# outbrain-inc/fwumious_wabbit

Measured on AMD Instinct MI355X. Metric: examples/sec + final log-loss, 30-field k=8 FFM, at 1/2/4/8 MI355X, higher is better.
Workload: dtype f32

## Files before the change

fwumious_wabbit_amd/_capi.py:

```python
import ctypes as C
import os

import numpy as np

_HERE = os.path.dirname(os.path.abspath(__file__))
LIB_PATH = os.environ.get("FWGPU_LIBRARY") or os.path.join(_HERE, "lib", "libfwgpu.so")

OK = 0
ERR_INVALID = 1
ERR_RANGE = 4
ERR_PARSE, ERR_IO, PARSE_FLUSH, PARSE_HOGWILD_LOAD = 6, 7, 100, 101
FFM_F32, FFM_F16_BUCKETS = 0, 1
OPT_SGD, OPT_ADAGRAD_FLEX, OPT_ADAGRAD_LUT = 100, 200, 300
WIRING_REGRESSOR, WIRING_FFM_ONLY = 0, 1
MODE_SEQUENTIAL, MODE_HOGWILD = 0, 1
TABLE_LR, TABLE_FFM_W, TABLE_FFM_ACC, TABLE_NN_W, TABLE_NN_ACC = 0, 1, 2, 3, 4
ROUTE_NONE, ROUTE_FUSED, ROUTE_HEAD_BATCHED, ROUTE_HEAD_BATCHED_REFUSED, ROUTE_PACKED, ROUTE_HOST_WALK = 0, 1, 2, 3, 4, 5
NN_INIT = {"xavier": 0, "hu": 1, "one": 2, "zero": 3}

CANDIDATE_INFO = np.dtype([("code", "<i4"), ("is_delta", "u1"), ("record_ok", "u1"), ("by_host", "u1"), ("pad", "u1"), ("n_lr", "<u4"),
                           ("n_ffm", "<u4")])
LR_ENTRY = np.dtype([("hash", "<u4"), ("value", "<f4"), ("combo_index", "<u4")])
FFM_ENTRY = np.dtype([("hash", "<u4"), ("value", "<f4"), ("contra_field_index", "<u4")])

# ... 106 lines not shown
        "fwgpu_dist_group_set_mode": [vp, i32],
        "fwgpu_dist_rank": [vp, P(i32), P(i32)],
        "fwgpu_dist_comm_count": [vp, P(i32)],
        "fwgpu_dist_ranges": [vp, P(u32), P(u32), P(u32), P(u32)],
        "fwgpu_dist_learn_sharded": [vp, P(TranslatorConfig), vp, vp, u32, vp],
        "fwgpu_dist_learn_sharded_batch": [vp, P(TranslatorConfig), vp],
        "fwgpu_dist_gather_tables": [vp],
        "fwgpu_dist_all_reduce_sum": [vp, vp, u64, vp],
        "fwgpu_dist_group_create": [vp, i32, P(vp)],
        "fwgpu_dist_group_free": [vp],
        "fwgpu_dist_group_learn_sharded": [vp, P(TranslatorConfig), vp, vp, u32, vp],
        "fwgpu_dist_group_gather_tables": [vp],
        "fwgpu_dist_learn_sparse": [vp, P(TranslatorConfig), vp, vp, u32, vp],
        "fwgpu_dist_learn_sparse_batch": [vp, P(TranslatorConfig), vp],
        "fwgpu_dist_sparse_last_rows": [vp, P(u32), P(u32)],
        "fwgpu_dist_group_learn_sparse": [vp, P(TranslatorConfig), vp, vp, vp, vp],
        "fwgpu_dist_group_learn_peer": [vp, P(TranslatorConfig), vp, vp, vp, vp, i32],
        "fwgpu_dist_peer_attach": [vp],
        "fwgpu_dist_owner_attach": [vp, u32, u32],
        "fwgpu_dist_learn_owner": [vp, P(TranslatorConfig), vp, vp, u32, vp, i32],
        "fwgpu_dist_group_learn_owner": [vp, P(TranslatorConfig), vp, vp, vp, vp, i32],
        "fwgpu_dist_group_learn_owner_stream": [vp, P(TranslatorConfig), vp, vp, vp, vp, vp, i32, u32, u32, u32],
        "fwgpu_dist_owner_stream_attach": [vp, u32, u32],
        "fwgpu_dist_learn_owner_stream": [vp, P(TranslatorConfig), vp, vp, u32, vp, i32, u32],
        "fwgpu_dist_learn_peer": [vp, P(TranslatorConfig), vp, vp, u32, vp, i32],
        "fwgpu_dist_learn_peer_batch": [vp, P(TranslatorConfig), vp, i32, vp],
        "fwgpu_dist_barrier": [vp],
        "fwgpu_split_create": [vp, u32, u32, P(vp)],
        "fwgpu_split_free": [vp],
        "fwgpu_learn_batch_sync": [vp, vp, vp, i32, vp],
        "fwgpu_serialized_len": [vp, P(u64)],
        "fwgpu_write_weights": [vp, vp, u64, P(u64)],
        "fwgpu_read_weights": [vp, vp, u64],
        "fwgpu_table_len": [vp, i32, P(u64)],
        "fwgpu_table_read": [vp, i32, u64, u64, vp],
        "fwgpu_table_write": [vp, i32, u64, u64, vp],
        "fwgpu_table_fill": [vp, i32, f32],
        "fwgpu_table_checksum": [vp, i32, P(u64)],
        "fwgpu_table_device_ptr": [vp, i32, P(vp)],
        "fwgpu_batch_create": [vp, vp, vp, vp, vp, vp, vp, u32, P(vp)],
        "fwgpu_batch_free": [vp],
        "fwgpu_batch_size": [vp, P(u32), P(u64), P(u64)],
        "fwgpu_learn_batch": [vp, vp, i32, i32, vp],
        "fwgpu_batch_predictions": [vp, vp, u32, vp],
        "fwgpu_batch_predictions_device": [vp, P(vp)],
        "fwgpu_translate": [P(TranslatorConfig), vp, u32, vp, u32, P(u32), vp, u32, P(u32), P(f32), P(f32)],
        "fwgpu_batch_from_records": [vp, P(TranslatorConfig), vp, vp, u32, P(vp)],
        "fwgpu_record_batch_create": [vp, P(TranslatorConfig), vp, vp, u32, P(vp)],
        "fwgpu_trainer_create": [vp, P(TranslatorConfig), u32, P(vp)],
        "fwgpu_digest_records": [vp, vp, vp, u32],
        "fwgpu_finish": [vp],
        "fwgpu_trainer_free": [vp],
        "fwgpu_trainer_examples_seen": [vp, P(u64)],
        "fwgpu_trainer_set_holdout": [vp, u64, i32],
        "fwgpu_trainer_predictions": [vp, vp, u64, P(u64)],
        "fwgpu_set_launch": [vp, u32, u32],
        "fwgpu_set_max_in_flight": [vp, u32],
        "fwgpu_delta_start": [vp, vp, vp, vp, u64, f32, vp],
        "fwgpu_delta_finish": [vp, vp, vp, vp, u64, vp],
        "fwgpu_debug_phase_ticks": [vp, i32, vp],
        "fwgpu_debug_placement": [vp, P(i32), P(C.c_float), P(C.c_float)],
        "fwgpu_debug_set_kernel_version": [vp, i32],
        "fwgpu_debug_set_option": [vp, i32, i32],
        "fwgpu_debug_last_route": [vp, P(i32)],
        "fwgpu_debug_head_inputs": [vp, vp, u64],
        "fwgpu_debug_coherence_probe": [i32, i32, u32, P(u32), P(u32)],
        "fwgpu_debug_head_gemm": [vp, vp, vp, i32, i32, i32, i32, i32, i32, i32, i32, i32, vp, vp, i32, i32, vp],
        "fwgpu_debug_sparse_reduce": [vp, u32, i32, vp, u32, u32, u32, vp, u32, vp, u32, vp, vp, vp, P(u32), vp],
        "fwgpu_debug_sparse_apply": [vp, vp, vp, u32, u32, i32, u32, u32, vp, vp, i32, f32, f32, vp, vp],
        "fwgpu_synth_records": [P(SynthConfig), u64, u32, vp, u64, vp, P(u64)],
        "fwgpu_debug_format_f32": [f32, C.c_char_p, u32],
        "fwgpu_vwmap_from_csv": [C.c_char_p, u64, P(vp)],
        "fwgpu_vwmap_from_json": [C.c_char_p, u64, P(vp)],
        "fwgpu_vwmap_to_json": [vp, vp, u64, P(u64)],
        "fwgpu_vwmap_lookup": [vp, C.c_char_p, u64, i32, P(u32), P(u32)],
        "fwgpu_parser_create": [vp, P(vp)],
        "fwgpu_parser_parse_line": [vp, C.c_char_p, u64, vp, u32, P(u32)],
        "fwgpu_parser_parse_with_prefix": [vp, C.c_char_p, u64, C.c_char_p, u64, vp, u32, P(u32)],
        "fwgpu_parse_prefix_create": [vp, C.c_char_p, u64, P(vp)],
        "fwgpu_parse_prefix_resumable": [vp],
        "fwgpu_parser_parse_after_prefix": [vp, vp, C.c_char_p, u64, vp, u32, P(u32)],
        "fwgpu_parse_prefix_is_record": [vp, vp, u32],
        "fwgpu_parser_parse_candidate": [vp, vp, C.c_char_p, u64, vp, u32, P(u32), P(i32)],
        "fwgpu_parser_parse_buffer": [vp, C.c_char_p, u64, vp, u64, vp, u64, P(u64), P(u64), P(u64)],
        "fwgpu_text_parser_create": [vp, i32, P(vp)],
        "fwgpu_text_parser_parse_buffer": [vp, C.c_char_p, u64, vp, u64, vp, u64, P(u64), P(u64), P(u64)],
        "fwgpu_text_parser_last_lines": [vp, P(u64), P(u64)],
        "fwgpu_text_parser_parse_candidates": [vp, vp, vp, P(TranslatorConfig), C.c_char_p, u64, u64, vp, u64, vp, vp, P(u64), P(u64)],
        "fwgpu_record_batch_from_text": [vp, P(TranslatorConfig), vp, C.c_char_p, u64, u64, P(vp), P(u64), P(u64)],
        "fwgpu_f32_from_text": [C.c_char_p, u64, P(f32), P(i32)],
        "fwgpu_mi_from_json": [C.c_char_p, u64, P(vp)],
        "fwgpu_mi_to_json": [vp, vp, u64, P(u64)],
        "fwgpu_mi_configs": [vp, i32, P(Config), P(TranslatorConfig), P(NNConfig)],
        "fwgpu_mi_set_inference": [vp, i32],
        "fwgpu_model_save": [C.c_char_p, vp, vp, vp, i32],
        "fwgpu_model_read_header": [C.c_char_p, P(vp), P(vp)],
        "fwgpu_model_load": [C.c_char_p, i32, i32, P(vp), P(vp), P(vp)],
        "fwgpu_model_load_packed": [C.c_char_p, i32, P(vp), P(vp), P(vp)],
        "fwgpu_ffm_storage": [vp, P(i32), P(u64)],
        "fwgpu_set_wiring": [vp, i32],
        "fwgpu_model_convert_inference": [C.c_char_p, C.c_char_p, i32],
        "fwgpu_quantize_ffm_weights": [vp, u64, vp, u64],
        "fwgpu_dequantize_ffm_weights": [vp, u64, vp],
        "fwgpu_trainer_digest_cache": [vp, vp, u64, P(u64)],
        "fwgpu_trainer_digest_text": [vp, vp, vp, C.c_char_p, u64, u32, P(u64), P(u64)],
        "fwgpu_parser_clone": [vp, P(vp)],
# ... 47 lines not shown
```

fwumious_wabbit_amd/csrc/fwgpu_internal.h:

```cpp
#pragma once

#include <hip/hip_runtime.h>
#include <stdint.h>

#include <memory>
#include <string>
#include <condition_variable>
#include <functional>
#include <mutex>
#include <thread>
#include <vector>

#include "fwgpu.h"

namespace fwgpu {

constexpr int kLutBits = 11;
constexpr int kLutSize = 1 << kLutBits;
constexpr uint32_t kFfmContraBufLen = 41472;

void set_error(const std::string &msg);
int fail(int code, const std::string &msg);
#define FWGPU_HIP(call)                                                                                  \
    do {                                                                                                 \
// ... 461 lines not shown
                 uint32_t *n_lr, uint32_t *n_ffm);
struct TextLines {
    const fwgpu_candidate_info *info = nullptr;
    const uint64_t *rec_off = nullptr;
    uint64_t n_lines = 0, n_words = 0;
};
int text_lines_scan(fwgpu_text_parser *tp, const fwgpu_parse_prefix *px, const fwgpu_block_cache *cache, const fwgpu_translator_config *t,
                    const char *text, uint64_t len, uint64_t piece_bytes, bool zero_word1, TextLines *out);
int text_lines_place(fwgpu_text_parser *tp, uint32_t *d_records);
int record_batch_alloc(fwgpu_regressor *r, const fwgpu_translator_config *t, uint32_t n_cap, uint64_t words_cap,
                       fwgpu_batch **out, bool host_mapped = false);
int mapped_batch_next_counter(fwgpu_batch *b, hipStream_t stream);
constexpr uint32_t kWorkRing = 1024;
struct RecordStats {
    uint32_t max_lr = 0, max_ffm = 0, max_rec = 0;
    uint64_t tot_lr = 0, tot_ffm = 0;
    void merge(const RecordStats &o) {
        max_lr = max_lr > o.max_lr ? max_lr : o.max_lr;
        max_ffm = max_ffm > o.max_ffm ? max_ffm : o.max_ffm;
        max_rec = max_rec > o.max_rec ? max_rec : o.max_rec;
        tot_lr += o.tot_lr;
        tot_ffm += o.tot_ffm;
    }
};
int count_records(const fwgpu_translator_config *t, const uint32_t *records, const uint64_t *rec_off, uint32_t n,
                  RecordStats *st);
int record_batch_upload(fwgpu_batch *b, const fwgpu_translator_config *t, const uint32_t *records,
                        const uint64_t *rec_off, uint32_t n, hipStream_t stream, const RecordStats *stats = nullptr);
uint32_t lr_hash_mask(uint32_t bit_precision);
uint32_t ffm_hash_mask(uint32_t ffm_bits, uint32_t ffm_k);
void lut_init(float *lut, float learning_rate, float power_t, float init_acc);
KernelParams make_params(const fwgpu_regressor *r, const fwgpu_batch *b, int update);
int refuse_packed(const fwgpu_regressor *r, const char *what);
int create_packed(const fwgpu_config *cfg, const float *lr_w, const uint8_t *blob, fwgpu_regressor **out);
int run_batch_peer(fwgpu_regressor *r, fwgpu_batch *b, int mode, int update, const PeerShards *d_shards, hipStream_t stream,
                   const PushRings *d_push = nullptr, uint32_t stream_consumers = 0, uint32_t device_share = 1, uint32_t stream_max_consumer_waves = 0, uint32_t n_ranks = 0);
hipError_t launch_rendezvous(uint32_t *counter, uint32_t n, uint32_t *met, hipStream_t stream);
hipError_t launch_owner_apply(const fwgpu_regressor *r, float *lr_base, const uint32_t *keys, const float *rows, uint32_t n_rows, const uint2 *lr_ent,
                              uint32_t n_lr, bool in_order, hipStream_t stream);
struct SplitRanges {
    uint32_t ffm_lo = 0, ffm_hi = 0xffffffffu, lr_lo = 0, lr_hi = 0xffffffffu, home_lo = 0, home_hi = 0xffffffffu;
};
struct OccBuffers {
    unsigned long long *ffm_key = nullptr, *lr_key = nullptr;
    uint2 *ffm_desc = nullptr, *lr_desc = nullptr;
};
int split_forward(fwgpu_regressor *r, fwgpu_batch *b, fwgpu_split *sp, int mode, const SplitRanges &rg, hipStream_t stream,
                  const OccBuffers *occ = nullptr, uint32_t *max_ffm = nullptr, uint32_t *max_lr = nullptr);
int split_mid(fwgpu_regressor *r, fwgpu_split *sp, uint32_t first, uint32_t n, float *d_pred, bool head, hipStream_t stream);
int split_update(fwgpu_regressor *r, fwgpu_batch *b, fwgpu_split *sp, int mode, const SplitRanges &rg, bool head, hipStream_t stream);
int head_step(fwgpu_regressor *r, fwgpu_split *sp, uint32_t first, uint32_t n, float *d_pred, bool update, hipStream_t stream);
void head_scratch_free(fwgpu_regressor *r);
uint32_t pick_grid(const fwgpu_regressor *r, const KernelParams &p, int mode, uint32_t threads);
}
```

fwumious_wabbit_amd/csrc/regressor.cpp:

```cpp
#include <math.h>
#include <string.h>

#include <algorithm>
#include <memory>

#include "fwgpu_internal.h"

#ifndef FWGPU_LR_THIN_DEFAULT
#define FWGPU_LR_THIN_DEFAULT 1
#endif
namespace fwgpu {

static thread_local std::string g_last_error;
void set_error(const std::string &msg) { g_last_error = msg; }
int fail(int code, const std::string &msg) {
    g_last_error = msg;
    return code;
}

int refuse_packed(const fwgpu_regressor *r, const char *what) {
    if (!r || !r->packed()) return FWGPU_OK;
    return fail(FWGPU_ERR_INVALID, std::string(what) + ": the regressor's FFM weights are packed f16 buckets (fwgpu_model_load_packed): it only predicts");
}

// ... 463 lines not shown
    if (!b->aligned4)
        return fail(FWGPU_ERR_INVALID, "packed regressor: an FFM entry's hash is not a multiple of 4 (rows must start where the translator's mask puts them: hash & fwgpu_ffm_hash_mask)");
    KernelParams p;
    uint32_t threads = 0;
    const int32_t kv = r->launch.kernel_version;
    r->launch.kernel_version = 0;
    int rc = prepare_launch(r, b, mode, 0, p, threads);
    r->launch.kernel_version = kv;
    if (rc) return rc;
    if (!example_kernel_is_resident(p, threads))
        return fail(FWGPU_ERR_INVALID, "packed regressor: the launch shape is not served (workgroups of at most 512 threads, at most 2048 FFM features per example)");
    const uint32_t grid = pick_grid(r, p, mode, threads);
    if (b->work_ring) {
        rc = mapped_batch_next_counter(b, stream);
        if (rc) return rc;
        p.work = b->work;
    } else {
        FWGPU_HIP(hipMemsetAsync(b->work, 0, sizeof(uint32_t), stream));
    }
    FWGPU_HIP(launch_packed_predict(p, r->q_increment, r->q_min, grid, threads, stream));
    return FWGPU_OK;
}

static int run_batch(fwgpu_regressor *r, fwgpu_batch *b, int mode, int update, hipStream_t stream, int32_t *route = nullptr) {
    if (route) *route = FWGPU_ROUTE_PACKED;
    if (r->packed()) return run_batch_packed(r, b, mode, update, stream);
    if (route) *route = FWGPU_ROUTE_NONE;
    if (b->n == 0) return FWGPU_OK;
    if (route) *route = FWGPU_ROUTE_HOST_WALK;
    if (b->host_copy) return run_batch_by_example(r, b, update, stream);
    if (route) *route = FWGPU_ROUTE_FUSED;
    if (head_predict_batched(r, b, mode, update)) {
        const int rcb = run_batch_head_predict(r, b, stream);
        if (route) *route = rcb == FWGPU_ERR_RANGE ? FWGPU_ROUTE_HEAD_BATCHED_REFUSED : FWGPU_ROUTE_HEAD_BATCHED;
        if (rcb != FWGPU_ERR_RANGE) {
            if (route && rcb == FWGPU_OK) r->pred_n = b->n;
            return rcb;
        }
    }
    KernelParams p;
    uint32_t threads = 0;
    int rc = prepare_launch(r, b, mode, update, p, threads);
    if (rc) return rc;
    const uint32_t grid = pick_grid(r, p, mode, threads);
    if (b->work_ring) {
        rc = mapped_batch_next_counter(b, stream);
        if (rc) return rc;
        p.work = b->work;
    } else {
        FWGPU_HIP(hipMemsetAsync(b->work, 0, sizeof(uint32_t), stream));
    }
    FWGPU_HIP(launch_example_kernel(p, r->cfg.optimizer, update != 0, grid, threads, stream));
    return FWGPU_OK;
}

static constexpr uint32_t kHeadPredictSlab = 32768;
static bool head_predict_batched(const fwgpu_regressor *r, const fwgpu_batch *b, int mode, int update) {
    static const bool env_off = getenv("FWGPU_HEAD_PREDICT_PER_EXAMPLE") != nullptr;
    const bool off = r->launch.head_predict >= 0 ? r->launch.head_predict == 0 : env_off;
    if (off || update || !r->nn.n_layers || mode != FWGPU_MODE_HOGWILD || b->n < 256 || b->emit_T) return false;
    const uint32_t k = r->cfg.ffm_k, R = k * r->cfg.ffm_num_fields;
    return k && k % 4 == 0 && b->aligned4 && (R <= 256 || (R <= 512 && 256 % k == 0)) && r->launch.kernel_version != 1;
}
static int run_batch_head_predict(fwgpu_regressor *r, fwgpu_batch *b, hipStream_t stream) {
    const uint32_t X = r->nn.X;
    if (r->pred_cap < b->n) {
        FWGPU_HIP(hipStreamSynchronize(stream));
        if (r->pred_x) (void)hipFree(r->pred_x);
        if (r->pred_yi) (void)hipFree(r->pred_yi);
        r->pred_x = r->pred_yi = nullptr;
        r->pred_cap = 0;
        if (hipMalloc((void **)&r->pred_x, (size_t)b->n * X * sizeof(float)) != hipSuccess || hipMalloc((void **)&r->pred_yi, (size_t)b->n * 2 * sizeof(float)) != hipSuccess) {
            (void)hipGetLastError();
            return fail(FWGPU_ERR_OOM, "predict batch with a deep head: no memory for the head's inputs");
        }
        r->pred_cap = b->n;
    }
    KernelParams p;
    uint32_t threads = 0;
    {
        p = make_params(r, b, 0);
        if (p.ctx_rec && b->max_rec < p.ctx_rec_len) return fail(FWGPU_ERR_RANGE, "candidate-only records: the batch's longest record does not include the context's");
        p.emit_x = 1;
        p.xbuf = r->pred_x;
        p.gbuf = r->pred_yi;
        threads = std::min<uint32_t>(r->launch.threads, 512);
        if ((uint64_t)p.max_ffm > 4ull * threads) return fail(FWGPU_ERR_RANGE, "an example has more than 2048 FFM features");
        resolve_row_mode(p, threads);
        if (example_kernel_lds_bytes(p, r->cfg.optimizer) > r->lds_per_cu) return fail(FWGPU_ERR_RANGE, "example does not fit the LDS");
    }
    if (b->work_ring) {
        int rc = mapped_batch_next_counter(b, stream);
        if (rc) return rc;
        p.work = b->work;
    } else {
        FWGPU_HIP(hipMemsetAsync(b->work, 0, sizeof(uint32_t), stream));
    }
    FWGPU_HIP(launch_example_kernel(p, r->cfg.optimizer, false, 0, threads, stream));
    fwgpu_split view;
    view.owner = r;
    view.d_x = r->pred_x;
    view.d_g = r->pred_yi;
    for (uint32_t first = 0; first < b->n; first += kHeadPredictSlab) {
        int rc = head_step(r, &view, first, std::min(kHeadPredictSlab, b->n - first), b->pred + first, false, stream);
        if (rc) return rc;
    }
// ... 1315 lines not shown
```

fwumious_wabbit_amd/csrc/trainer.cpp:

```cpp
#include <string.h>

#include <string>

#include <algorithm>
#include <memory>
#include <chrono>
#include <thread>

#include "fwgpu_internal.h"

using namespace fwgpu;

struct fwgpu_trainer {
    fwgpu_regressor *r = nullptr;
    uint32_t micro_batch = 0;
    std::vector<uint32_t> combo_off, combo_ns, field_off, field_ns;
    std::vector<uint8_t> combo_f32, field_f32;
    std::vector<float> combo_weight;
    fwgpu_translator_config t{};
    uint32_t *rec[2] = {nullptr, nullptr};
    uint64_t rec_used[2] = {0, 0}, rec_cap[2] = {0, 0};
    std::vector<uint64_t> off[2];
    RecordStats stats[2];
    unsigned host_threads = 1;
    fwgpu_batch *dev[2] = {nullptr, nullptr};
    hipEvent_t done[2] = {nullptr, nullptr};
    hipEvent_t uploaded[2] = {nullptr, nullptr};
    hipStream_t copy_stream = nullptr;
    bool in_flight[2] = {false, false};
    int cur = 0;
    hipStream_t stream = nullptr;
    uint64_t seen = 0;
    uint64_t holdout_after = 0;
    bool testonly = false;
    bool slot_predict[2] = {false, false};
    uint32_t slot_n[2] = {0, 0};
    float *pred_host[2] = {nullptr, nullptr};
    uint32_t pred_cap[2] = {0, 0};
    std::vector<float> preds;
    std::unique_ptr<uint32_t[]> cache_words[2];
    std::unique_ptr<uint64_t[]> cache_off[2];
    uint64_t cache_off_cap = 0;
    Workers copy_pool, parse_pool;
};

static bool predict_mode(const fwgpu_trainer *tr) {
    return tr->testonly || (tr->holdout_after && tr->seen + 1 >= tr->holdout_after);
}

static int retire(fwgpu_trainer *tr, int c) {
    if (!tr->in_flight[c]) return FWGPU_OK;
    FWGPU_HIP(hipEventSynchronize(tr->done[c]));
    tr->in_flight[c] = false;
    if (tr->slot_predict[c]) tr->preds.insert(tr->preds.end(), tr->pred_host[c], tr->pred_host[c] + tr->slot_n[c]);
    tr->slot_predict[c] = false;
    return FWGPU_OK;
}

static int flush(fwgpu_trainer *tr, bool predict = false) {
    const int c = tr->cur;
    const uint32_t n = (uint32_t)(tr->off[c].size() - 1);
    if (n == 0) return FWGPU_OK;
    fwgpu_regressor *r = tr->r;
    FWGPU_HIP(hipSetDevice(r->device));
    int rrc = retire(tr, c);
    if (rrc) return rrc;
    const uint64_t words = tr->rec_used[c];
    fwgpu_batch *b = tr->dev[c];
    if (!b || b->n_cap < n || b->words_cap < words) {
        if (b) fwgpu_batch_free(b);
        tr->dev[c] = nullptr;
        int rc = record_batch_alloc(r, &tr->t, std::max(n, tr->micro_batch), words * 3 / 2 + 4096, &tr->dev[c]);
        if (rc) return rc;
        b = tr->dev[c];
    }
    int rc = record_batch_upload(b, &tr->t, tr->rec[c], tr->off[c].data(), n, tr->copy_stream, &tr->stats[c]);
    if (rc) return rc;
    if ((rc = record_batch_host_copy_if_oversize(r, &tr->t, b, tr->rec[c], tr->off[c].data(), n))) return rc;
    FWGPU_HIP(hipEventRecord(tr->uploaded[c], tr->copy_stream));
    FWGPU_HIP(hipStreamWaitEvent(tr->stream, tr->uploaded[c], 0));
    rc = fwgpu_learn_batch(r, b, FWGPU_MODE_HOGWILD, predict ? 0 : 1, tr->stream);
    if (rc) return rc;
    if (predict) {
        if (tr->pred_cap[c] < n) {
            if (tr->pred_host[c]) (void)hipHostFree(tr->pred_host[c]);
            tr->pred_host[c] = nullptr;
            FWGPU_HIP(hipHostMalloc((void **)&tr->pred_host[c], (size_t)std::max(n, tr->micro_batch) * 4, hipHostMallocDefault));
            tr->pred_cap[c] = std::max(n, tr->micro_batch);
        }
        FWGPU_HIP(hipMemcpyAsync(tr->pred_host[c], b->pred, (size_t)n * 4, hipMemcpyDeviceToHost, tr->stream));
    }
    tr->slot_predict[c] = predict;
    tr->slot_n[c] = n;
    FWGPU_HIP(hipEventRecord(tr->done[c], tr->stream));
    tr->in_flight[c] = true;
    tr->cur ^= 1;
    const int c2 = tr->cur;
    rrc = retire(tr, c2);
    if (rrc) return rrc;
    tr->rec_used[c2] = 0;
    tr->off[c2].assign(1, 0);
    tr->stats[c2] = RecordStats();
    return FWGPU_OK;
}

extern "C" {

int fwgpu_trainer_create(fwgpu_regressor *r, const fwgpu_translator_config *t, uint32_t micro_batch, fwgpu_trainer **out) {
    if (!r || !t || !out) return fail(FWGPU_ERR_INVALID, "NULL argument");
    if (micro_batch == 0) return fail(FWGPU_ERR_INVALID, "micro_batch must be > 0");
    if (int rcp = refuse_packed(r, "trainer_create")) return rcp;
    int crc = check_translator(r, t);
    if (crc) return crc;
    std::unique_ptr<fwgpu_trainer> tr(new fwgpu_trainer());
    tr->r = r;
    tr->micro_batch = micro_batch;
    tr->combo_off.assign(t->combo_off, t->combo_off + t->n_combos + 1);
    const uint32_t ncm = t->n_combos ? t->combo_off[t->n_combos] : 0;
    tr->combo_ns.assign(t->combo_ns, t->combo_ns + ncm);
    tr->combo_f32.assign(t->combo_ns_f32, t->combo_ns_f32 + ncm);
    tr->combo_weight.assign(t->combo_weight, t->combo_weight + t->n_combos);
    tr->field_off.assign(t->field_off, t->field_off + t->n_fields + 1);
    const uint32_t nfm = t->n_fields ? t->field_off[t->n_fields] : 0;
    tr->field_ns.assign(t->field_ns, t->field_ns + nfm);
    tr->field_f32.assign(t->field_ns_f32, t->field_ns_f32 + nfm);
    tr->t = *t;
    tr->t.combo_off = tr->combo_off.data();
    tr->t.combo_ns = tr->combo_ns.data();
    tr->t.combo_ns_f32 = tr->combo_f32.data();
    tr->t.combo_weight = tr->combo_weight.data();
    tr->t.field_off = tr->field_off.data();
    tr->t.field_ns = tr->field_ns.data();
    tr->t.field_ns_f32 = tr->field_f32.data();
    tr->off[0].assign(1, 0);
    tr->off[1].assign(1, 0);
    tr->host_threads = std::max(1u, std::thread::hardware_concurrency());
    FWGPU_HIP(hipSetDevice(r->device));
    FWGPU_HIP(hipStreamCreateWithFlags(&tr->stream, hipStreamNonBlocking));
    FWGPU_HIP(hipStreamCreateWithFlags(&tr->copy_stream, hipStreamNonBlocking));
    FWGPU_HIP(hipEventCreateWithFlags(&tr->uploaded[0], hipEventDisableTiming));
    FWGPU_HIP(hipEventCreateWithFlags(&tr->uploaded[1], hipEventDisableTiming));
    FWGPU_HIP(hipEventCreateWithFlags(&tr->done[0], hipEventDisableTiming));
    FWGPU_HIP(hipEventCreateWithFlags(&tr->done[1], hipEventDisableTiming));
    *out = tr.release();
    return FWGPU_OK;
}

int fwgpu_digest_records(fwgpu_trainer *tr, const uint32_t *records, const uint64_t *rec_off, uint32_t n) {
    if (!tr || (n && (!records || !rec_off))) return fail(FWGPU_ERR_INVALID, "NULL argument");
    uint32_t i = 0;
    while (i < n) {
        const int c = tr->cur;
        const uint32_t have = (uint32_t)(tr->off[c].size() - 1);
        uint32_t take = std::min<uint32_t>(n - i, tr->micro_batch - have);
        const bool predicting = predict_mode(tr);
        if (!predicting && tr->holdout_after) {
            const uint64_t until = tr->holdout_after - 1 - tr->seen;
            if (take > until) take = (uint32_t)until;
        }
        const uint64_t w0 = rec_off[i], w1 = rec_off[i + take];
        const uint64_t base = tr->rec_used[c];
        if (base + (w1 - w0) > tr->rec_cap[c]) {
            const uint64_t ncap = std::max<uint64_t>((base + (w1 - w0)) * 2, 1u << 20);
            uint32_t *nbuf = nullptr;
            FWGPU_HIP(hipSetDevice(tr->r->device));
            FWGPU_HIP(hipHostMalloc((void **)&nbuf, ncap * 4, hipHostMallocDefault));
            if (base) memcpy(nbuf, tr->rec[c], base * 4);
            if (tr->rec[c]) (void)hipHostFree(tr->rec[c]);
            tr->rec[c] = nbuf;
            tr->rec_cap[c] = ncap;
        }
        {
            const unsigned T = take >= 4096 ? std::min<unsigned>(tr->host_threads, 8) : 1;
            std::vector<RecordStats> st(T);
            std::vector<int> rcs(T, FWGPU_OK);
            std::vector<std::string> msgs(T);
            auto work = [&](unsigned k) {
                const uint32_t a = i + (uint32_t)((uint64_t)take * k / T), e = i + (uint32_t)((uint64_t)take * (k + 1) / T);
                memcpy(tr->rec[c] + base + (rec_off[a] - w0), records + rec_off[a], (rec_off[e] - rec_off[a]) * 4);
                rcs[k] = count_records(&tr->t, records, rec_off + a, e - a, &st[k]);
                if (rcs[k]) msgs[k] = fwgpu_last_error();
            };
            tr->copy_pool.run(T, work);
            for (unsigned k = 0; k < T; k++) {
                if (rcs[k]) return fail(rcs[k], msgs[k]);
                tr->stats[c].merge(st[k]);
            }
        }
        tr->rec_used[c] = base + (w1 - w0);
        for (uint32_t j = 1; j <= take; j++) tr->off[c].push_back(base + (rec_off[i + j] - w0));
        tr->seen += take;
        i += take;
        if (tr->off[c].size() - 1 >= tr->micro_batch || (!predicting && predict_mode(tr))) {
            int rc = flush(tr, predicting);
// ... 193 lines not shown
    auto ms = [](std::chrono::steady_clock::time_point a, std::chrono::steady_clock::time_point b) {
        return std::chrono::duration<double, std::milli>(b - a).count();
    };
    while (have) {
        bool go_on = true;
        double t_digest = 0.0;
        const auto t0 = now();
        std::thread dg([&] {
            go_on = digest_slices(cur, rc, msg);
            t_digest = ms(t0, now());
        });
        bool parsed_next = false;
        if (pos < len) {
            const uint64_t e = chunk_end(pos);
            parse_range(pos, e, next);
            pos = e;
            parsed_next = true;
        }
        const double t_parse = ms(t0, now());
        dg.join();
        if (timing) fprintf(stderr, "[digest_text] chunk: parse of the next %.2f ms, digest of this one %.2f ms, both %.2f ms\n", t_parse, t_digest, ms(t0, now()));
        if (!go_on || !parsed_next) break;
        cur.swap(next);
    }
    if (rc != FWGPU_OK && rc != FWGPU_PARSE_FLUSH && rc != FWGPU_PARSE_HOGWILD_LOAD) rc = fail(rc, msg);
    if (n_examples) *n_examples = done;
    if (consumed) *consumed = used;
    return rc;
}

int fwgpu_trainer_set_holdout(fwgpu_trainer *tr, uint64_t holdout_after, int testonly) {
    if (!tr) return fail(FWGPU_ERR_INVALID, "NULL trainer");
    if (tr->off[tr->cur].size() > 1) return fail(FWGPU_ERR_INVALID, "set the hold-out before digesting (or right after fwgpu_finish)");
    tr->holdout_after = holdout_after;
    tr->testonly = testonly != 0;
    return FWGPU_OK;
}

int fwgpu_trainer_predictions(fwgpu_trainer *tr, float *out, uint64_t cap, uint64_t *n) {
    if (!tr || !n) return fail(FWGPU_ERR_INVALID, "NULL argument");
    *n = tr->preds.size();
    if (!out) return FWGPU_OK;
    if (cap < tr->preds.size()) return fail(FWGPU_ERR_RANGE, "buffer too small for the predictions");
    if (!tr->preds.empty()) memcpy(out, tr->preds.data(), tr->preds.size() * 4);
    return FWGPU_OK;
}

int fwgpu_finish(fwgpu_trainer *tr) {
    if (!tr) return fail(FWGPU_ERR_INVALID, "NULL trainer");
    const bool last_predict = tr->testonly || (tr->holdout_after && tr->seen >= tr->holdout_after);
    int rc = flush(tr, last_predict);
    if (rc) return rc;
    FWGPU_HIP(hipSetDevice(tr->r->device));
    FWGPU_HIP(hipStreamSynchronize(tr->stream));
    rc = retire(tr, tr->cur);
    if (rc) return rc;
    rc = retire(tr, tr->cur ^ 1);
    if (rc) return rc;
    return FWGPU_OK;
}

int fwgpu_trainer_free(fwgpu_trainer *tr) {
    if (!tr) return FWGPU_OK;
    (void)hipSetDevice(tr->r->device);
    if (tr->stream) (void)hipStreamSynchronize(tr->stream);
    for (int i = 0; i < 2; i++) {
        if (tr->dev[i]) fwgpu_batch_free(tr->dev[i]);
        if (tr->rec[i]) (void)hipHostFree(tr->rec[i]);
        if (tr->pred_host[i]) (void)hipHostFree(tr->pred_host[i]);
        if (tr->done[i]) (void)hipEventDestroy(tr->done[i]);
    }
    if (tr->stream) (void)hipStreamDestroy(tr->stream);
    if (tr->copy_stream) (void)hipStreamDestroy(tr->copy_stream);
    for (int i = 0; i < 2; i++)
        if (tr->uploaded[i]) (void)hipEventDestroy(tr->uploaded[i]);
    delete tr;
    return FWGPU_OK;
}

int fwgpu_trainer_examples_seen(const fwgpu_trainer *tr, uint64_t *n) {
    if (!tr || !n) return fail(FWGPU_ERR_INVALID, "NULL argument");
    *n = tr->seen;
    return FWGPU_OK;
}

}
```

fwumious_wabbit_amd/regressor.py:

```python
import ctypes as C
from dataclasses import dataclass, field
from typing import List, Optional, Tuple

import numpy as np

from . import _capi as capi
from ._capi import FFM_ENTRY, LR_ENTRY, check, ptr


class Optimizer:
    SGD = capi.OPT_SGD
    AdagradFlex = capi.OPT_ADAGRAD_FLEX
    AdagradLUT = capi.OPT_ADAGRAD_LUT


@dataclass
class NamespaceDescriptor:
    namespace_index: int
    namespace_format_f32: bool = False


@dataclass
class FeatureComboDesc:
    namespace_descriptors: List[NamespaceDescriptor]
# ... 456 lines not shown
        self.translator = FeatureBufferTranslator(model_instance)
        self.h = C.c_void_p()
        check(capi.lib().fwgpu_trainer_create(regressor.h, C.byref(self.translator.c), micro_batch, C.byref(self.h)))

    def digest_example(self, feature_buffer):
        rec = np.ascontiguousarray(feature_buffer, dtype=np.uint32)
        off = np.array([0, len(rec)], dtype=np.uint64)
        check(capi.lib().fwgpu_digest_records(self.h, ptr(rec), ptr(off), 1))

    def digest_records(self, records, rec_off):
        records = np.ascontiguousarray(records, dtype=np.uint32)
        rec_off = np.ascontiguousarray(rec_off, dtype=np.uint64)
        check(capi.lib().fwgpu_digest_records(self.h, ptr(records), ptr(rec_off), len(rec_off) - 1))

    def set_holdout(self, holdout_after=0, testonly=False):
        check(capi.lib().fwgpu_trainer_set_holdout(self.h, holdout_after, int(testonly)))

    def predictions(self) -> np.ndarray:
        n = C.c_uint64()
        check(capi.lib().fwgpu_trainer_predictions(self.h, None, 0, C.byref(n)))
        out = np.zeros(n.value, dtype=np.float32)
        check(capi.lib().fwgpu_trainer_predictions(self.h, ptr(out), out.size, C.byref(n)))
        return out

    def digest_cache(self, cache, max_records=0) -> int:
        n = C.c_uint64()
        check(capi.lib().fwgpu_trainer_digest_cache(self.h, cache.h, max_records, C.byref(n)))
        return n.value

    def digest_text(self, parser, text: bytes, cache=None, threads=0):
        n, used = C.c_uint64(), C.c_uint64()
        rc = capi.lib().fwgpu_trainer_digest_text(self.h, parser.h, cache.h if cache is not None else None, text, len(text),
                                                  threads, C.byref(n), C.byref(used))
        if rc not in (capi.OK, capi.PARSE_FLUSH, capi.PARSE_HOGWILD_LOAD):
            check(rc)
        return n.value, used.value, rc

    def digest_file(self, parser, filename: str, cache=None, threads=0):
        n = C.c_uint64()
        rc = capi.lib().fwgpu_trainer_digest_file(self.h, parser.h, cache.h if cache is not None else None, filename.encode(),
                                                  threads, C.byref(n))
        if rc not in (capi.OK, capi.PARSE_FLUSH, capi.PARSE_HOGWILD_LOAD):
            check(rc)
        return n.value, rc

    def block_until_workers_finished(self):
        check(capi.lib().fwgpu_finish(self.h))

    def examples_seen(self):
        n = C.c_uint64(0)
        check(capi.lib().fwgpu_trainer_examples_seen(self.h, C.byref(n)))
        return n.value

    def close(self):
        if self.h:
            capi.lib().fwgpu_trainer_free(self.h)
            self.h = C.c_void_p()

    def __del__(self):
        try:
            self.close()
        except Exception:
            pass


def synth_records(n_namespaces, mean_extra, zipf_s, ids_per_ns, p_weighted, seed, first_example, n):
    L = capi.lib()
    cfg = capi.SynthConfig(n_namespaces, mean_extra, zipf_s, ids_per_ns, p_weighted, seed)
    nw = C.c_uint64(0)
    rec_off = np.zeros(n + 1, dtype=np.uint64)
    check(L.fwgpu_synth_records(C.byref(cfg), first_example, n, None, 0, ptr(rec_off), C.byref(nw)))
    records = np.zeros(nw.value, dtype=np.uint32)
    check(L.fwgpu_synth_records(C.byref(cfg), first_example, n, ptr(records), nw.value, ptr(rec_off), C.byref(nw)))
    return records, rec_off
```

include/fwgpu.h:

```cpp
#ifndef FWGPU_H
#define FWGPU_H

#include <stddef.h>
#include <stdint.h>

#ifdef __cplusplus
extern "C" {
#endif

#define FWGPU_ABI_VERSION 1

enum {
    FWGPU_OK = 0,
    FWGPU_ERR_INVALID = 1,
    FWGPU_ERR_DEVICE = 2,
    FWGPU_ERR_OOM = 3,
    FWGPU_ERR_RANGE = 4,
    FWGPU_ERR_FORMAT = 5,
    FWGPU_ERR_PARSE = 6,
    FWGPU_ERR_IO = 7,
    FWGPU_ERR_PEER = 8,
    FWGPU_PARSE_FLUSH = 100,
    FWGPU_PARSE_HOGWILD_LOAD = 101
};
// ... 127 lines not shown

typedef struct fwgpu_dist fwgpu_dist;
typedef struct fwgpu_dist_group fwgpu_dist_group;
int fwgpu_dist_unique_id(uint8_t *id, uint64_t cap );
int fwgpu_dist_init(fwgpu_regressor *r, const uint8_t *unique_id, int rank, int n_ranks, fwgpu_dist **out);
int fwgpu_dist_free(fwgpu_dist *d);
int fwgpu_dist_set_mode(fwgpu_dist *d, int mode);
int fwgpu_dist_group_set_mode(fwgpu_dist_group *g, int mode);
int fwgpu_dist_owner_attach(fwgpu_dist *d, uint32_t max_rows, uint32_t max_lr);
int fwgpu_dist_learn_owner(fwgpu_dist *d, const fwgpu_translator_config *t, const uint32_t *records, const uint64_t *rec_off, uint32_t n,
                           float *predictions, int update);
int fwgpu_dist_group_learn_owner(fwgpu_dist_group *g, const fwgpu_translator_config *t, const uint32_t *const *records,
                                 const uint64_t *const *rec_off, const uint32_t *n, float *const *predictions, int update);
int fwgpu_dist_group_learn_owner_stream(fwgpu_dist_group *g, const fwgpu_translator_config *t, const uint32_t *const *records, const uint64_t *const *rec_off,
                                        const uint32_t *n, fwgpu_batch *const *batches, float *const *predictions, int update, uint32_t log2_rows,
                                        uint32_t log2_lr, uint32_t consumer_workgroups);
int fwgpu_dist_owner_stream_attach(fwgpu_dist *d, uint32_t log2_rows, uint32_t log2_lr);
int fwgpu_dist_learn_owner_stream(fwgpu_dist *d, const fwgpu_translator_config *t, const uint32_t *records, const uint64_t *rec_off, uint32_t n,
                                  float *predictions, int update, uint32_t consumer_workgroups);
int fwgpu_dist_rank(const fwgpu_dist *d, int *rank, int *n_ranks);
int fwgpu_dist_comm_count(const fwgpu_dist *d, int *count);
int fwgpu_dist_ranges(const fwgpu_dist *d, uint32_t *ffm_lo, uint32_t *ffm_hi, uint32_t *lr_lo, uint32_t *lr_hi);
int fwgpu_dist_learn_sharded(fwgpu_dist *d, const fwgpu_translator_config *t, const uint32_t *records, const uint64_t *rec_off,
                             uint32_t n, float *predictions);
int fwgpu_dist_learn_sharded_batch(fwgpu_dist *d, const fwgpu_translator_config *t, fwgpu_batch *b);
int fwgpu_dist_gather_tables(fwgpu_dist *d);
int fwgpu_dist_all_reduce_sum(fwgpu_dist *d, float *device_buf, uint64_t count, void *hip_stream);
int fwgpu_dist_group_create(fwgpu_regressor *const *regressors, int n_ranks, fwgpu_dist_group **out);
int fwgpu_dist_group_free(fwgpu_dist_group *g);
int fwgpu_dist_group_learn_sharded(fwgpu_dist_group *g, const fwgpu_translator_config *t, const uint32_t *const *records,
                                   const uint64_t *const *rec_off, uint32_t n, float *const *predictions);
int fwgpu_dist_group_gather_tables(fwgpu_dist_group *g);
int fwgpu_dist_learn_sparse(fwgpu_dist *d, const fwgpu_translator_config *t, const uint32_t *records, const uint64_t *rec_off,
                            uint32_t n, float *predictions);
int fwgpu_dist_learn_sparse_batch(fwgpu_dist *d, const fwgpu_translator_config *t, fwgpu_batch *b);
int fwgpu_dist_sparse_last_rows(const fwgpu_dist *d, uint32_t *ffm_rows, uint32_t *lr_rows);
int fwgpu_dist_group_learn_sparse(fwgpu_dist_group *g, const fwgpu_translator_config *t, const uint32_t *const *records,
                                  const uint64_t *const *rec_off, const uint32_t *n, float *const *predictions);
int fwgpu_dist_group_learn_peer(fwgpu_dist_group *g, const fwgpu_translator_config *t, const uint32_t *const *records,
                                const uint64_t *const *rec_off, const uint32_t *n, float *const *predictions, int update);
int fwgpu_dist_peer_attach(fwgpu_dist *d);
int fwgpu_dist_learn_peer(fwgpu_dist *d, const fwgpu_translator_config *t, const uint32_t *records, const uint64_t *rec_off, uint32_t n,
                          float *predictions, int update);
int fwgpu_dist_learn_peer_batch(fwgpu_dist *d, const fwgpu_translator_config *t, fwgpu_batch *b, int update, void *hip_stream);
int fwgpu_dist_barrier(fwgpu_dist *d);


int fwgpu_trainer_create(fwgpu_regressor *r, const fwgpu_translator_config *t, uint32_t micro_batch,
                         fwgpu_trainer **out);
int fwgpu_digest_records(fwgpu_trainer *tr, const uint32_t *records, const uint64_t *rec_off, uint32_t n);
int fwgpu_finish(fwgpu_trainer *tr);
int fwgpu_trainer_free(fwgpu_trainer *tr);
int fwgpu_trainer_examples_seen(const fwgpu_trainer *tr, uint64_t *n);
int fwgpu_trainer_set_holdout(fwgpu_trainer *tr, uint64_t holdout_after, int testonly);
int fwgpu_trainer_predictions(fwgpu_trainer *tr, float *out, uint64_t cap, uint64_t *n);

int fwgpu_set_launch(fwgpu_regressor *r, uint32_t threads, uint32_t workgroups_per_cu);
int fwgpu_set_wiring(fwgpu_regressor *r, int wiring);
int fwgpu_set_max_in_flight(fwgpu_regressor *r, uint32_t n_examples);

int fwgpu_delta_start(const void *table, const void *snapshot, void *local_delta, void *summed_delta, uint64_t n_floats,
                      float scale, void *stream);
int fwgpu_delta_finish(void *table, void *snapshot, const void *local_delta, const void *summed_delta, uint64_t n_floats,
                       void *stream);

int fwgpu_debug_phase_ticks(fwgpu_regressor *r, int enable, uint64_t *out16);
int fwgpu_debug_placement(const fwgpu_regressor *r, int *tries, float *ms_fastest, float *ms_slowest);
int fwgpu_debug_set_kernel_version(fwgpu_regressor *r, int version);
int fwgpu_debug_set_option(fwgpu_regressor *r, int option, int value);
#define FWGPU_ROUTE_NONE 0
#define FWGPU_ROUTE_FUSED 1
#define FWGPU_ROUTE_HEAD_BATCHED 2
#define FWGPU_ROUTE_HEAD_BATCHED_REFUSED 3
#define FWGPU_ROUTE_PACKED 4
#define FWGPU_ROUTE_HOST_WALK 5
int fwgpu_debug_last_route(const fwgpu_regressor *r, int *route);
int fwgpu_debug_head_inputs(fwgpu_regressor *r, float *out, uint64_t n_floats);
int fwgpu_debug_format_f32(float v, char *buf, uint32_t cap);
int fwgpu_debug_coherence_probe(int device, int use_sc1, uint32_t iters, uint32_t *stale_words, uint32_t *timeouts);
int fwgpu_debug_head_gemm(const float *A, const float *B, float *C, int M, int N, int K, int lda, int ldb, int ldc, int ta, int tb, int epilogue,
                          const float *bias, float *aux, int relu, int tiled, void *stream);
int fwgpu_debug_sparse_reduce(const void *keys, uint32_t n, int key_bits, const void *desc, uint32_t max_entries, uint32_t R, uint32_t k,
                              const float *split, uint32_t split_len, const float *selfw, uint32_t selfw_stride, const float *gbuf, uint32_t *bk_key,
                              float *bk_rows, uint32_t *count, void *stream);
int fwgpu_debug_sparse_apply(const uint32_t *all_key, const float *all_rows, const uint32_t *counts, uint32_t n_ranks, uint32_t stride, int key_bits,
                             uint32_t R, uint32_t k4, float *w, float *acc, int optimizer, float rate, float minus_power_t, const float *lut,
                             void *stream);

typedef struct fwgpu_vwmap fwgpu_vwmap;
int fwgpu_vwmap_from_csv(const char *csv, uint64_t len, fwgpu_vwmap **out);
int fwgpu_vwmap_from_json(const char *json, uint64_t len, fwgpu_vwmap **out);
void fwgpu_vwmap_free(fwgpu_vwmap *vw);
uint32_t fwgpu_vwmap_num_namespaces(const fwgpu_vwmap *vw);
uint32_t fwgpu_vwmap_num_entries(const fwgpu_vwmap *vw);
int fwgpu_vwmap_to_json(const fwgpu_vwmap *vw, char *buf, uint64_t cap, uint64_t *len);
int fwgpu_vwmap_lookup(const fwgpu_vwmap *vw, const char *name, uint64_t len, int verbose, uint32_t *index,
                       uint32_t *is_f32);

typedef struct fwgpu_parser fwgpu_parser;
int fwgpu_parser_create(const fwgpu_vwmap *vw, fwgpu_parser **out);
void fwgpu_parser_free(fwgpu_parser *p);
int fwgpu_parser_parse_line(fwgpu_parser *p, const char *line, uint64_t len, uint32_t *out, uint32_t cap, uint32_t *n_words);
int fwgpu_parser_parse_with_prefix(fwgpu_parser *p, const char *prefix, uint64_t prefix_len, const char *line, uint64_t len,
                                   uint32_t *out, uint32_t cap, uint32_t *n_words);
typedef struct fwgpu_parse_prefix fwgpu_parse_prefix;
int fwgpu_parse_prefix_create(fwgpu_parser *p, const char *prefix, uint64_t len, fwgpu_parse_prefix **out);
// ... 89 lines not shown
```

Measured before the change: 6.786 million.

## Run trainer micro-batches on two compute streams so hogwild learns overlap

Replaces the single compute stream plus separate copy stream with one stream per double-buffer slot, doing the upload and learn kernel on the same slot stream. When the learn launch is eligible (hogwild-concurrent, no NN, no host caps), the next batch's kernel is no longer ordered behind the previous one, so two micro-batches can run on the GPU at once. This removes the serialization between consecutive batches, at the cost of more racy hogwild updates, which could shift the final log-loss. It also adds a debug counter for overlapped versus ordered launches, and an environment switch to fall back to ordered launches.

```diff
diff --git a/fwumious_wabbit_amd/_capi.py b/fwumious_wabbit_amd/_capi.py
--- a/fwumious_wabbit_amd/_capi.py
+++ b/fwumious_wabbit_amd/_capi.py
@@ -182,6 +182,7 @@
         "fwgpu_finish": [vp],
         "fwgpu_trainer_free": [vp],
         "fwgpu_trainer_examples_seen": [vp, P(u64)],
+        "fwgpu_debug_trainer_launches": [vp, P(u64), P(u64)],
         "fwgpu_trainer_set_holdout": [vp, u64, i32],
         "fwgpu_trainer_predictions": [vp, vp, u64, P(u64)],
         "fwgpu_set_launch": [vp, u32, u32],
diff --git a/fwumious_wabbit_amd/csrc/fwgpu_internal.h b/fwumious_wabbit_amd/csrc/fwgpu_internal.h
--- a/fwumious_wabbit_amd/csrc/fwgpu_internal.h
+++ b/fwumious_wabbit_amd/csrc/fwgpu_internal.h
@@ -537,4 +537,5 @@
 int head_step(fwgpu_regressor *r, fwgpu_split *sp, uint32_t first, uint32_t n, float *d_pred, bool update, hipStream_t stream);
 void head_scratch_free(fwgpu_regressor *r);
 uint32_t pick_grid(const fwgpu_regressor *r, const KernelParams &p, int mode, uint32_t threads);
+bool learn_launch_may_overlap(fwgpu_regressor *r, fwgpu_batch *b);
 }
diff --git a/fwumious_wabbit_amd/csrc/regressor.cpp b/fwumious_wabbit_amd/csrc/regressor.cpp
--- a/fwumious_wabbit_amd/csrc/regressor.cpp
+++ b/fwumious_wabbit_amd/csrc/regressor.cpp
@@ -539,6 +539,18 @@
     }
     FWGPU_HIP(launch_example_kernel(p, r->cfg.optimizer, update != 0, grid, threads, stream));
     return FWGPU_OK;
+}
+
+bool learn_launch_may_overlap(fwgpu_regressor *r, fwgpu_batch *b) {
+    if (r->packed() || r->nn.n_layers || r->d_ticks || b->host_copy || b->work_ring || b->n == 0) return false;
+    KernelParams p;
+    uint32_t threads = 0;
+    const std::string keep = fwgpu_last_error();
+    if (prepare_launch(r, b, FWGPU_MODE_HOGWILD, 1, p, threads) != FWGPU_OK) {
+        set_error(keep);
+        return false;
+    }
+    return p.concurrent && !p.host_grid_cap && !p.host_wgs_cap;
 }
 
 static constexpr uint32_t kHeadPredictSlab = 32768;
diff --git a/fwumious_wabbit_amd/csrc/trainer.cpp b/fwumious_wabbit_amd/csrc/trainer.cpp
--- a/fwumious_wabbit_amd/csrc/trainer.cpp
+++ b/fwumious_wabbit_amd/csrc/trainer.cpp
@@ -25,11 +25,12 @@
     unsigned host_threads = 1;
     fwgpu_batch *dev[2] = {nullptr, nullptr};
     hipEvent_t done[2] = {nullptr, nullptr};
-    hipEvent_t uploaded[2] = {nullptr, nullptr};
-    hipStream_t copy_stream = nullptr;
     bool in_flight[2] = {false, false};
     int cur = 0;
-    hipStream_t stream = nullptr;
+    hipStream_t compute[2] = {nullptr, nullptr};
+    bool slot_ordered[2] = {false, false};
+    bool two_streams = true;
+    uint64_t n_overlapped = 0, n_ordered = 0;
     uint64_t seen = 0;
     uint64_t holdout_after = 0;
     bool testonly = false;
@@ -74,12 +75,19 @@
         if (rc) return rc;
         b = tr->dev[c];
     }
-    int rc = record_batch_upload(b, &tr->t, tr->rec[c], tr->off[c].data(), n, tr->copy_stream, &tr->stats[c]);
+    hipStream_t stream = tr->compute[c];
+    int rc = record_batch_upload(b, &tr->t, tr->rec[c], tr->off[c].data(), n, stream, &tr->stats[c]);
     if (rc) return rc;
     if ((rc = record_batch_host_copy_if_oversize(r, &tr->t, b, tr->rec[c], tr->off[c].data(), n))) return rc;
-    FWGPU_HIP(hipEventRecord(tr->uploaded[c], tr->copy_stream));
-    FWGPU_HIP(hipStreamWaitEvent(tr->stream, tr->uploaded[c], 0));
-    rc = fwgpu_learn_batch(r, b, FWGPU_MODE_HOGWILD, predict ? 0 : 1, tr->stream);
+    const bool overlap = tr->two_streams && !predict && learn_launch_may_overlap(r, b);
+    if (tr->in_flight[c ^ 1] && (!overlap || tr->slot_ordered[c ^ 1])) {
+        FWGPU_HIP(hipStreamWaitEvent(stream, tr->done[c ^ 1], 0));
+    }
+    if (overlap)
+        tr->n_overlapped++;
+    else
+        tr->n_ordered++;
+    rc = fwgpu_learn_batch(r, b, FWGPU_MODE_HOGWILD, predict ? 0 : 1, stream);
     if (rc) return rc;
     if (predict) {
         if (tr->pred_cap[c] < n) {
@@ -88,11 +96,12 @@
             FWGPU_HIP(hipHostMalloc((void **)&tr->pred_host[c], (size_t)std::max(n, tr->micro_batch) * 4, hipHostMallocDefault));
             tr->pred_cap[c] = std::max(n, tr->micro_batch);
         }
-        FWGPU_HIP(hipMemcpyAsync(tr->pred_host[c], b->pred, (size_t)n * 4, hipMemcpyDeviceToHost, tr->stream));
+        FWGPU_HIP(hipMemcpyAsync(tr->pred_host[c], b->pred, (size_t)n * 4, hipMemcpyDeviceToHost, stream));
     }
     tr->slot_predict[c] = predict;
     tr->slot_n[c] = n;
-    FWGPU_HIP(hipEventRecord(tr->done[c], tr->stream));
+    FWGPU_HIP(hipEventRecord(tr->done[c], stream));
+    tr->slot_ordered[c] = !overlap;
     tr->in_flight[c] = true;
     tr->cur ^= 1;
     const int c2 = tr->cur;
@@ -136,10 +145,12 @@
     tr->off[1].assign(1, 0);
     tr->host_threads = std::max(1u, std::thread::hardware_concurrency());
     FWGPU_HIP(hipSetDevice(r->device));
-    FWGPU_HIP(hipStreamCreateWithFlags(&tr->stream, hipStreamNonBlocking));
-    FWGPU_HIP(hipStreamCreateWithFlags(&tr->copy_stream, hipStreamNonBlocking));
-    FWGPU_HIP(hipEventCreateWithFlags(&tr->uploaded[0], hipEventDisableTiming));
-    FWGPU_HIP(hipEventCreateWithFlags(&tr->uploaded[1], hipEventDisableTiming));
+    FWGPU_HIP(hipStreamCreateWithFlags(&tr->compute[0], hipStreamNonBlocking));
+    FWGPU_HIP(hipStreamCreateWithFlags(&tr->compute[1], hipStreamNonBlocking));
+    {
+        const char *env = getenv("FWGPU_TRAINER_STREAMS");
+        tr->two_streams = !(env && env[0] == '1');
+    }
     FWGPU_HIP(hipEventCreateWithFlags(&tr->done[0], hipEventDisableTiming));
     FWGPU_HIP(hipEventCreateWithFlags(&tr->done[1], hipEventDisableTiming));
     *out = tr.release();
@@ -439,7 +450,6 @@
     int rc = flush(tr, last_predict);
     if (rc) return rc;
     FWGPU_HIP(hipSetDevice(tr->r->device));
-    FWGPU_HIP(hipStreamSynchronize(tr->stream));
     rc = retire(tr, tr->cur);
     if (rc) return rc;
     rc = retire(tr, tr->cur ^ 1);
@@ -450,17 +460,16 @@
 int fwgpu_trainer_free(fwgpu_trainer *tr) {
     if (!tr) return FWGPU_OK;
     (void)hipSetDevice(tr->r->device);
-    if (tr->stream) (void)hipStreamSynchronize(tr->stream);
+    for (int i = 0; i < 2; i++)
+        if (tr->compute[i]) (void)hipStreamSynchronize(tr->compute[i]);
     for (int i = 0; i < 2; i++) {
         if (tr->dev[i]) fwgpu_batch_free(tr->dev[i]);
         if (tr->rec[i]) (void)hipHostFree(tr->rec[i]);
         if (tr->pred_host[i]) (void)hipHostFree(tr->pred_host[i]);
         if (tr->done[i]) (void)hipEventDestroy(tr->done[i]);
     }
-    if (tr->stream) (void)hipStreamDestroy(tr->stream);
-    if (tr->copy_stream) (void)hipStreamDestroy(tr->copy_stream);
     for (int i = 0; i < 2; i++)
-        if (tr->uploaded[i]) (void)hipEventDestroy(tr->uploaded[i]);
+        if (tr->compute[i]) (void)hipStreamDestroy(tr->compute[i]);
     delete tr;
     return FWGPU_OK;
 }
@@ -471,4 +480,11 @@
     return FWGPU_OK;
 }
 
-}
+int fwgpu_debug_trainer_launches(const fwgpu_trainer *tr, uint64_t *overlapped, uint64_t *ordered) {
+    if (!tr) return fail(FWGPU_ERR_INVALID, "NULL trainer");
+    if (overlapped) *overlapped = tr->n_overlapped;
+    if (ordered) *ordered = tr->n_ordered;
+    return FWGPU_OK;
+}
+
+}
diff --git a/fwumious_wabbit_amd/regressor.py b/fwumious_wabbit_amd/regressor.py
--- a/fwumious_wabbit_amd/regressor.py
+++ b/fwumious_wabbit_amd/regressor.py
@@ -532,6 +532,11 @@
         check(capi.lib().fwgpu_trainer_examples_seen(self.h, C.byref(n)))
         return n.value
 
+    def launches(self):
+        a, b = C.c_uint64(0), C.c_uint64(0)
+        check(capi.lib().fwgpu_debug_trainer_launches(self.h, C.byref(a), C.byref(b)))
+        return a.value, b.value
+
     def close(self):
         if self.h:
             capi.lib().fwgpu_trainer_free(self.h)
diff --git a/include/fwgpu.h b/include/fwgpu.h
--- a/include/fwgpu.h
+++ b/include/fwgpu.h
@@ -203,6 +203,7 @@
 int fwgpu_finish(fwgpu_trainer *tr);
 int fwgpu_trainer_free(fwgpu_trainer *tr);
 int fwgpu_trainer_examples_seen(const fwgpu_trainer *tr, uint64_t *n);
+int fwgpu_debug_trainer_launches(const fwgpu_trainer *tr, uint64_t *overlapped, uint64_t *ordered);
 int fwgpu_trainer_set_holdout(fwgpu_trainer *tr, uint64_t holdout_after, int testonly);
 int fwgpu_trainer_predictions(fwgpu_trainer *tr, float *out, uint64_t cap, uint64_t *n);
 
```

Result: no change. 6.789 million (median of 3 runs) (+0.1%).
